# UW-RoboSoccer/tsid_control

Measured on AMD Instinct MI355X. Metric: env-steps/sec (whole node), higher is better.
Workload: dtype f64

## Files before the change

### tsid_control_amd/csrc/tsidb_common.hpp

```cpp
#pragma once
#include <hip/hip_runtime.h>
#include <stdint.h>

#ifdef TSIDB_STAMPS
constexpr int NSTAMP = 48;
__device__ unsigned long long g_stamp[8192][NSTAMP];
#define TSIDB_STAMP(k) do { if (threadIdx.x == 0 && blockIdx.x < 8192) g_stamp[blockIdx.x][k] = __builtin_amdgcn_s_memtime(); } while (0)
#define TSIDB_LAP_INIT() unsigned long long lap_t_ = __builtin_amdgcn_s_memtime()
#define TSIDB_LAP(k) do { unsigned long long n_ = __builtin_amdgcn_s_memtime(); if (threadIdx.x == 0 && blockIdx.x < 8192) g_stamp[blockIdx.x][k] += n_ - lap_t_; lap_t_ = n_; } while (0)
#define TSIDB_LAP_ZERO(k) do { if (threadIdx.x == 0 && blockIdx.x < 8192) g_stamp[blockIdx.x][k] = 0; } while (0)
#else
#define TSIDB_STAMP(k) do { } while (0)
#define TSIDB_LAP_INIT() do { } while (0)
#define TSIDB_LAP(k) do { } while (0)
#define TSIDB_LAP_ZERO(k) do { } while (0)
#endif

#ifndef TSIDB_TOPOLOGY_HEADER
#define TSIDB_TOPOLOGY_HEADER "tsidb_topology.hpp"
#endif
#include TSIDB_TOPOLOGY_HEADER

namespace tsidb {

// ... 159 lines not shown
  s = (q & 2) ? -s0 : s0;
  c = ((q + 1) & 2) ? -c0 : c0;
}

__device__ __forceinline__ int env_of_block(int b, int n) {
  constexpr int NXCD = 8;
  const int x = b % NXCD, i = b / NXCD, q = n / NXCD, r = n % NXCD;
  return x * q + (x < r ? x : r) + i;
}

constexpr double SIM_STATE_BOUND = 1e6;
template <typename T> struct Eps;
template <> struct Eps<double> { static constexpr double v = 2.220446049250313e-16; static constexpr double inf = 1e300; };
template <> struct Eps<float> { static constexpr float v = 1.1920929e-07f; static constexpr float inf = 1e30f; };

template <int CTRL, int ROW_MASK> __device__ __forceinline__ float dpp_mov(float v) {
  return __builtin_bit_cast(float, __builtin_amdgcn_update_dpp(0, __builtin_bit_cast(int, v), CTRL, ROW_MASK, 0xf, true));
}
template <int CTRL, int ROW_MASK> __device__ __forceinline__ double dpp_mov(double v) {
  const long long b = __builtin_bit_cast(long long, v);
  const int lo = __builtin_amdgcn_update_dpp(0, (int)(b & 0xffffffffLL), CTRL, ROW_MASK, 0xf, true);
  const int hi = __builtin_amdgcn_update_dpp(0, (int)(b >> 32), CTRL, ROW_MASK, 0xf, true);
  return __builtin_bit_cast(double, ((long long)hi << 32) | (unsigned int)lo);
}
__device__ __forceinline__ float lane63(float v) {
  return __builtin_bit_cast(float, __builtin_amdgcn_readlane(__builtin_bit_cast(int, v), 63));
}
__device__ __forceinline__ int lane63(int v) { return __builtin_amdgcn_readlane(v, 63); }
__device__ __forceinline__ double lane63(double v) {
  const long long b = __builtin_bit_cast(long long, v);
  const int lo = __builtin_amdgcn_readlane((int)(b & 0xffffffffLL), 63), hi = __builtin_amdgcn_readlane((int)(b >> 32), 63);
  return __builtin_bit_cast(double, ((long long)hi << 32) | (unsigned int)lo);
}
template <typename T> __device__ __forceinline__ T wave_sum(T v) {
  v += dpp_mov<0xB1, 0xf>(v);
  v += dpp_mov<0x4E, 0xf>(v);
  v += dpp_mov<0x141, 0xf>(v);
  v += dpp_mov<0x140, 0xf>(v);
  v += dpp_mov<0x142, 0xa>(v);
  v += dpp_mov<0x143, 0xc>(v);
  return lane63(v);
}
template <typename T> __device__ __forceinline__ void wave_sum3(T &a, T &b, T &c) {
#define TSIDB_SUM3_STEP(CTRL, MASK)                                                                  \
  {                                                                                                  \
    const T ta = dpp_mov<CTRL, MASK>(a), tb = dpp_mov<CTRL, MASK>(b), tc = dpp_mov<CTRL, MASK>(c);   \
    a += ta; b += tb; c += tc;                                                                       \
  }
  TSIDB_SUM3_STEP(0xB1, 0xf) TSIDB_SUM3_STEP(0x4E, 0xf) TSIDB_SUM3_STEP(0x141, 0xf) TSIDB_SUM3_STEP(0x140, 0xf)
  TSIDB_SUM3_STEP(0x142, 0xa) TSIDB_SUM3_STEP(0x143, 0xc)
#undef TSIDB_SUM3_STEP
  a = lane63(a); b = lane63(b); c = lane63(c);
}
template <typename T> __device__ __forceinline__ T bperm(T v, int src_lane) {
  if constexpr (sizeof(T) == 4) {
    return __builtin_bit_cast(T, __builtin_amdgcn_ds_bpermute(src_lane << 2, __builtin_bit_cast(int, v)));
  } else {
    const long long b = __builtin_bit_cast(long long, v);
    const int lo = __builtin_amdgcn_ds_bpermute(src_lane << 2, (int)(b & 0xffffffffLL));
    const int hi = __builtin_amdgcn_ds_bpermute(src_lane << 2, (int)(b >> 32));
    return __builtin_bit_cast(T, ((long long)hi << 32) | (unsigned int)lo);
  }
}
template <typename T> __device__ __forceinline__ T subtree_sum32(T v, int last) {
  T p = v;
  p += dpp_mov<0x111, 0xf>(p);
  p += dpp_mov<0x112, 0xf>(p);
  p += dpp_mov<0x114, 0xf>(p);
  p += dpp_mov<0x118, 0xf>(p);
  p += dpp_mov<0x142, 0xa>(p);
  return (bperm(p, last) - p) + v;
}

__device__ __forceinline__ int wave_sum_int(int v) {
  v += __builtin_amdgcn_update_dpp(0, v, 0xB1, 0xf, 0xf, true);
  v += __builtin_amdgcn_update_dpp(0, v, 0x4E, 0xf, 0xf, true);
  v += __builtin_amdgcn_update_dpp(0, v, 0x141, 0xf, 0xf, true);
  v += __builtin_amdgcn_update_dpp(0, v, 0x140, 0xf, 0xf, true);
  v += __builtin_amdgcn_update_dpp(0, v, 0x142, 0xa, 0xf, true);
  v += __builtin_amdgcn_update_dpp(0, v, 0x143, 0xc, 0xf, true);
  return __builtin_amdgcn_readlane(v, 63);
}

template <int CTRL, int ROW_MASK, typename T> __device__ __forceinline__ T dpp_min_step(T v) {
  T w;
  if constexpr (sizeof(T) == 4) {
    w = __builtin_bit_cast(T, __builtin_amdgcn_update_dpp(__builtin_bit_cast(int, v), __builtin_bit_cast(int, v), CTRL, ROW_MASK, 0xf, false));
  } else {
    const long long b = __builtin_bit_cast(long long, v);
    const int lo = __builtin_amdgcn_update_dpp((int)(b & 0xffffffffLL), (int)(b & 0xffffffffLL), CTRL, ROW_MASK, 0xf, false);
    const int hi = __builtin_amdgcn_update_dpp((int)(b >> 32), (int)(b >> 32), CTRL, ROW_MASK, 0xf, false);
    w = __builtin_bit_cast(T, ((long long)hi << 32) | (unsigned int)lo);
  }
  return w < v ? w : v;
}
template <typename T> __device__ __forceinline__ T wave_min(T v) {
  v = dpp_min_step<0xB1, 0xf>(v);
  v = dpp_min_step<0x4E, 0xf>(v);
  v = dpp_min_step<0x141, 0xf>(v);
  v = dpp_min_step<0x140, 0xf>(v);
  v = dpp_min_step<0x142, 0xa>(v);
  v = dpp_min_step<0x143, 0xc>(v);
  return lane63(v);
}
template <typename T> __device__ __forceinline__ void wave_argmin(T &v, int &i) {
  const T vmin = wave_min(v);
  i = wave_min<int>(v == vmin ? i : 0x7fffffff);
  v = vmin;
}
__device__ __forceinline__ int wave_min_int(int v) { return wave_min<int>(v); }

template <typename T> __device__ __forceinline__ void quat_to_R(T x, T y, T z, T w, T *R) {
  T n = T(1) / sqrt(x * x + y * y + z * z + w * w);
  x *= n; y *= n; z *= n; w *= n;
  R[0] = 1 - 2 * (y * y + z * z); R[1] = 2 * (x * y - w * z); R[2] = 2 * (x * z + w * y);
  R[3] = 2 * (x * y + w * z); R[4] = 1 - 2 * (x * x + z * z); R[5] = 2 * (y * z - w * x);
  R[6] = 2 * (x * z - w * y); R[7] = 2 * (y * z + w * x); R[8] = 1 - 2 * (x * x + y * y);
}

template <typename T> __device__ __forceinline__ void yo_mul(const T *Y, const T *X, T *f) {
  T wxh[3], hxl[3];
  cross3(X + 3, Y + 1, wxh);
  cross3(Y + 1, X, hxl);
  f[0] = Y[0] * X[0] + wxh[0];
  f[1] = Y[0] * X[1] + wxh[1];
  f[2] = Y[0] * X[2] + wxh[2];
  f[3] = Y[4] * X[3] + Y[5] * X[4] + Y[6] * X[5] + hxl[0];
  f[4] = Y[5] * X[3] + Y[7] * X[4] + Y[8] * X[5] + hxl[1];
  f[5] = Y[6] * X[3] + Y[8] * X[4] + Y[9] * X[5] + hxl[2];
}
template <typename T> __device__ __forceinline__ void cross_mm(const T *a, const T *b, T *o) {
  T t1[3], t2[3], t3[3];
  cross3(a + 3, b, t1); cross3(a, b + 3, t2); cross3(a + 3, b + 3, t3);
#pragma unroll
  for (int i = 0; i < 3; i++) { o[i] = t1[i] + t2[i]; o[3 + i] = t3[i]; }
}
template <typename T> __device__ __forceinline__ void cross_mf(const T *v, const T *f, T *o) {
  T t1[3], t2[3], t3[3];
  cross3(v + 3, f, t1); cross3(v + 3, f + 3, t2); cross3(v, f, t3);
#pragma unroll
  for (int i = 0; i < 3; i++) { o[i] = t1[i]; o[3 + i] = t2[i] + t3[i]; }
}

__device__ __forceinline__ void wave_sync() {
  __builtin_amdgcn_fence(__ATOMIC_RELEASE, "wavefront");
  __builtin_amdgcn_wave_barrier();
  __builtin_amdgcn_fence(__ATOMIC_ACQUIRE, "wavefront");
}

template <typename T>
__device__ __forceinline__ void tree_forward(int lane, int n, int up0, int up1, int up2, const int (&chn)[7], T *bufA, T *bufB,
                                             T *sq, int sq_stride, T *cb, int cb_stride, T (&R)[9], T (&p)[3], T qd,
                                             T (&S)[6], T (&V)[6], T (&A)[6]) {
  const bool on = lane < n;
  if (on) {
#pragma unroll
    for (int i = 0; i < 9; i++) bufA[lane * 12 + i] = R[i];
#pragma unroll
    for (int i = 0; i < 3; i++) bufA[lane * 12 + 9 + i] = p[i];
  }
  __syncthreads();
#pragma unroll
  for (int r = 0; r < 3; r++) {
    const int u = r == 0 ? up0 : (r == 1 ? up1 : up2);
    const T *src = (r & 1) ? bufB : bufA;
    T *dst = (r & 1) ? bufA : bufB;
// ... 112 lines not shown
```

### tsid_control_amd/csrc/tsidb_sim.hpp

```cpp
#pragma once
#include "tsidb_common.hpp"
#include "tsidb_tick.hpp"

namespace tsidb {

constexpr int LDM = 27;
constexpr int NEWTON_INCR_MAX = 8;

template <typename T>
struct Floor {
  T n[3], t1[3], t2[3], d;
};

template <typename T>
struct SimLds {
  Floor<T> fl;
  T S[NV][6];
  union {
    struct { T V[NB][6], A[NB][6], f[NB][6], Yc[NB][10]; };
    struct {
      T K[NB][21];
      T hn[MAXHH][3];
      int hb1[MAXHH];
    };
  };
  T M[NV * LDM];
  union {
    struct {
      T R[NB][9], p[NB][3];
      int fcand[64];
      int pcand[128];
      T terr[20];
      T scen[NG][4];
      T hn_s[MAXHH][3];
      int hb1_s[MAXHH];
    };
    T H[NV * LDM];
    T Wc[MAXCON][21];
  };
  T qpos[NQ], qvel[NV];
  T xv[NV];
  int cbody[MAXCON], cvert[MAXCON], cgeom[MAXCON];
  T ctq[CONDIM > 3 ? MAXCON : 1][3];
  unsigned anc[NB];
  T cr[MAXCON][3], cdist[MAXCON], cfv[MAXCON][3];
  int xch[4];
  unsigned char cchain[MAXCON][8];
};
static_assert(sizeof(SimLds<double>) <= 20480, "k_sim must fit 8 workgroups per CU");

template <int NW> __device__ __forceinline__ void wsync() {
  if constexpr (NW == 1) __syncthreads();
  else wave_sync();
}

__device__ __forceinline__ int sym_idx(int i, int j) {
  const int a = i < j ? i : j, b = i < j ? j : i;
  return a * 6 - a * (a - 1) / 2 + (b - a);
}

template <typename T, bool DENSE>
__device__ __forceinline__ T chol26_solve(T (&a)[NV], T rhs, int lane, bool &spd) {
  int ln = lane;
  asm volatile("" : "+v"(ln));
  int notspd = 0;
  T rd[NV];
#pragma unroll
  for (int t = 0; t < NV; t++) {
    const int k = NV - 1 - t;
    const T akk = rdlane(a[k], k);
    notspd = akk > 0 ? notspd : 1;
    asm volatile("" : "+v"(notspd));
    const T rk = rsqrt_t(akk > 0 ? akk : T(1));
    rd[k] = rk;
    T uik = ln < k ? a[k] * rk : (ln == k ? akk * rk : T(0));
    a[k] = uik;
    int jl = -1;
#pragma unroll
    for (int j0 = 0; j0 < k; j0 += 4) {
      const bool p0 = DENSE || ((MJ_DOFANC[k] >> j0) & 1u), p1 = j0 + 1 < k && (DENSE || ((MJ_DOFANC[k] >> (j0 + 1)) & 1u)),
                 p2 = j0 + 2 < k && (DENSE || ((MJ_DOFANC[k] >> (j0 + 2)) & 1u)), p3 = j0 + 3 < k && (DENSE || ((MJ_DOFANC[k] >> (j0 + 3)) & 1u));
      if (!(p0 || p1 || p2 || p3)) continue;
      const T u0 = p0 ? rdlane(uik, j0) : T(0), u1 = p1 ? rdlane(uik, j0 + 1) : T(0), u2 = p2 ? rdlane(uik, j0 + 2) : T(0),
              u3 = p3 ? rdlane(uik, j0 + 3) : T(0);
      if (jl >= 0) asm volatile("" : "+v"(uik), "+v"(a[jl]) : "s"(u0), "s"(u1), "s"(u2), "s"(u3));
      else asm volatile("" : "+v"(uik) : "s"(u0), "s"(u1), "s"(u2), "s"(u3));
      if (p0) { a[j0] -= uik * u0; jl = j0; }
      if (p1) { a[j0 + 1] -= uik * u1; jl = j0 + 1; }
      if (p2) { a[j0 + 2] -= uik * u2; jl = j0 + 2; }
      if (p3) { a[j0 + 3] -= uik * u3; jl = j0 + 3; }
    }
  }
  spd = notspd == 0;
#pragma unroll
  for (int k = 0; k < NV; k++) asm volatile("" : "+v"(a[k]));
  T acc = rhs, y[NV];
#pragma unroll
  for (int t = 0; t < NV; t++) {
    const int k = NV - 1 - t;
    y[k] = rdlane(acc, k) * rd[k];
    acc -= a[k] * y[k];
  }
  T xs[NV], x = 0;
#pragma unroll
  for (int t = NV - 1; t >= 0; t--) {
    const int k = NV - 1 - t;
    T s0 = y[k], s1 = 0, ak = a[k];
#pragma unroll
    for (int i0 = 0; i0 < k; i0 += 4) {
      const bool p0 = DENSE || ((MJ_DOFANC[k] >> i0) & 1u), p1 = i0 + 1 < k && (DENSE || ((MJ_DOFANC[k] >> (i0 + 1)) & 1u)),
                 p2 = i0 + 2 < k && (DENSE || ((MJ_DOFANC[k] >> (i0 + 2)) & 1u)), p3 = i0 + 3 < k && (DENSE || ((MJ_DOFANC[k] >> (i0 + 3)) & 1u));
      if (!(p0 || p1 || p2 || p3)) continue;
      const T u0 = p0 ? rdlane(ak, i0) : T(0), u1 = p1 ? rdlane(ak, i0 + 1) : T(0), u2 = p2 ? rdlane(ak, i0 + 2) : T(0),
              u3 = p3 ? rdlane(ak, i0 + 3) : T(0);
      asm volatile("" : "+v"(ak), "+v"(s0), "+v"(s1) : "s"(u0), "s"(u1), "s"(u2), "s"(u3));
      if (p0) s0 -= u0 * xs[i0];
      if (p1) s1 -= u1 * xs[i0 + 1];
      if (p2) s0 -= u2 * xs[i0 + 2];
      if (p3) s1 -= u3 * xs[i0 + 3];
    }
    xs[k] = (s0 + s1) * rd[k];
    if (ln == k) x = xs[k];
  }
  return x;
}

template <typename T>
__device__ __noinline__ T chol26_dense(T (&a)[NV], T rhs, int lane, bool &spd) { return chol26_solve<T, true>(a, rhs, lane, spd); }

template <typename T>
__device__ __forceinline__ void chol26_factor(T (&a)[NV], T &rdv, int lane, bool &spd) {
  int ln = lane;
  asm volatile("" : "+v"(ln));
  int notspd = 0;
  rdv = 0;
#pragma unroll
  for (int t = 0; t < NV; t++) {
    const int k = NV - 1 - t;
    const T akk = rdlane(a[k], k);
    notspd = akk > 0 ? notspd : 1;
    asm volatile("" : "+v"(notspd));
    const T rk = rsqrt_t(akk > 0 ? akk : T(1));
    rdv = ln == k ? rk : rdv;
    T uik = ln < k ? a[k] * rk : (ln == k ? akk * rk : T(0));
    a[k] = uik;
    int jl = -1;
#pragma unroll
    for (int j0 = 0; j0 < k; j0 += 4) {
      const bool p0 = (MJ_DOFANC[k] >> j0) & 1u, p1 = j0 + 1 < k && ((MJ_DOFANC[k] >> (j0 + 1)) & 1u),
                 p2 = j0 + 2 < k && ((MJ_DOFANC[k] >> (j0 + 2)) & 1u), p3 = j0 + 3 < k && ((MJ_DOFANC[k] >> (j0 + 3)) & 1u);
      if (!(p0 || p1 || p2 || p3)) continue;
      const T u0 = p0 ? rdlane(uik, j0) : T(0), u1 = p1 ? rdlane(uik, j0 + 1) : T(0), u2 = p2 ? rdlane(uik, j0 + 2) : T(0),
              u3 = p3 ? rdlane(uik, j0 + 3) : T(0);
      if (jl >= 0) asm volatile("" : "+v"(uik), "+v"(a[jl]) : "s"(u0), "s"(u1), "s"(u2), "s"(u3));
      else asm volatile("" : "+v"(uik) : "s"(u0), "s"(u1), "s"(u2), "s"(u3));
      if (p0) { a[j0] -= uik * u0; jl = j0; }
      if (p1) { a[j0 + 1] -= uik * u1; jl = j0 + 1; }
      if (p2) { a[j0 + 2] -= uik * u2; jl = j0 + 2; }
      if (p3) { a[j0 + 3] -= uik * u3; jl = j0 + 3; }
    }
  }
  spd = notspd == 0;
#pragma unroll
  for (int k = 0; k < NV; k++) asm volatile("" : "+v"(a[k]));
}

template <typename T>
__device__ __forceinline__ T chol26_subst(const T (&a)[NV], const T *Up, T rdv, T rhs, int lane) {
  int ln = lane;
  asm volatile("" : "+v"(ln));
  T b[NV];
#pragma unroll
  for (int i = 0; i < NV; i++) b[i] = lane < NV ? Up[i * LDM + lane] : T(0);
  T acc = rhs, yv = 0;
#pragma unroll
  for (int t = 0; t < NV; t++) {
    const int k = NV - 1 - t;
    const T yl = acc * rdv;
    const T yk = rdlane(yl, k);
    yv = ln == k ? yl : yv;
    acc -= a[k] * yk;
  }
  acc = yv;
  T x = 0;
#pragma unroll
  for (int i = 0; i < NV; i++) {
    const T xl = acc * rdv;
    const T xi = rdlane(xl, i);
    x = ln == i ? xl : x;
    acc -= b[i] * xi;
  }
  return x;
}

template <typename T>
__device__ __forceinline__ bool chol26_rank1(T (&a)[NV], T &rdv, T xv, T sigma, unsigned long long chain, int lane) {
  bool ok = true;
#pragma unroll
  for (int t = 0; t < NV; t++) {
    const int k = NV - 1 - t;
    if (ok && ((chain >> k) & 1ull)) {
      const T s = rdlane(xv * rdv, k);
      const T q = T(1) + sigma * s * s;
      if (!(q > (sizeof(T) == 8 ? T(1e-10) : T(1e-5)))) ok = false;
      else {
        const T ic = rsqrt_t(q), c = q * ic;
        const T un = (a[k] + sigma * s * xv) * ic;
        xv = lane == k ? T(0) : c * xv - s * un;
        a[k] = un;
        rdv = lane == k ? rdv * ic : rdv;
      }
    }
  }
  return ok;
}

template <typename T> __device__ __forceinline__ T mulM(const SimLds<T> &L, const T *x, int lane) {
  T s = 0, s1 = 0, s2 = 0, s3 = 0;
  if (lane < NV) {
    const T *Mr = &L.M[lane * LDM];
#pragma unroll
    for (int j = 0; j < NV; j += 4) {
      s += Mr[j] * x[j];
      if (j + 1 < NV) s1 += Mr[j + 1] * x[j + 1];
      if (j + 2 < NV) s2 += Mr[j + 2] * x[j + 2];
      if (j + 3 < NV) s3 += Mr[j + 3] * x[j + 3];
    }
  }
  return (s + s1) + (s2 + s3);
}

template <typename T> __device__ __forceinline__ void make_frame(const T *n, T *t1, T *t2) {
  T t[3] = {0, 0, 0};
  if (fabs(n[1]) < T(0.5)) t[1] = 1; else t[2] = 1;
  const T dn = dot3(n, t);
  T nn = 0;
#pragma unroll
  for (int i = 0; i < 3; i++) { t1[i] = t[i] - dn * n[i]; nn += t1[i] * t1[i]; }
  nn = T(1) / sqrt(nn);
#pragma unroll
  for (int i = 0; i < 3; i++) t1[i] *= nn;
  cross3(n, t1, t2);
// ... 1676 lines not shown
```

### tsid_control_amd/csrc/tsidb_tick.hpp

```cpp
#pragma once
#include "tsidb_common.hpp"

namespace tsidb {

constexpr int NAS = 34;

template <typename T>
struct KinScratch {
  T S[NV][6], fR[2][9], fp[2][3];
  union {
    T f[NJ][6];
    struct { T arhs[4][6], acomr[3], apost[NA], aamr[3]; };
  };
  T Yc[NJ][10];
  union {
    struct { T R[NJ][9], p[NJ][3], V[NJ][6], A[NJ][6]; };
    struct { T Jf[12 * LDF], Jcom[3 * LDF], Jam[3 * LDF]; };
  };
};

template <typename T>
struct ActiveSetLds {
  T Ra[NAS * (NAS + 1) / 2 + 2];
  T Rinv[NAS + 2];
  T s[160];
  T actp[3][NA];
  int slot[NAS + 2], A[NAS + 2], Aold[NAS + 2];
  unsigned char cstate[160];
};

template <typename T>
struct TickLds {
  union {
    KinScratch<T> k;
    ActiveSetLds<T> as;
  };
  T Dyn[NV * LDD];
  T h[NV];
  T x[NVAR];
  T oMf[2][12];
  T vf[2][6], af[2][6];
  T com[3], vcom[3], acomd[3];
  T Lam[3], dLam[3];
  T qs[NQ], vs[NV];
  int act[2];
};
static_assert(sizeof(ActiveSetLds<double>) <= sizeof(KinScratch<double>), "active-set state must fit the scratch region");
static_assert(sizeof(TickLds<double>) <= 20480, "k_tick must fit 8 workgroups per CU");

template <typename T> __device__ __forceinline__ T bcast(T v, int src) { return __shfl(v, src, WAVE); }

__device__ __forceinline__ float rdlane(float v, int src) {
  return __builtin_bit_cast(float, __builtin_amdgcn_readlane(__builtin_bit_cast(int, v), src));
}
__device__ __forceinline__ double rdlane(double v, int src) {
  long long b = __builtin_bit_cast(long long, v);
  int lo = __builtin_amdgcn_readlane((int)(b & 0xffffffffLL), src);
  int hi = __builtin_amdgcn_readlane((int)(b >> 32), src);
  return __builtin_bit_cast(double, ((long long)hi << 32) | (unsigned int)lo);
}


template <typename T>
__device__ __forceinline__ void rbd_terms(const DevModel<T> &m, TickLds<T> &L, int lane) {
  KinScratch<T> &K = L.k;
  const T GZ = T(9.81);
  TSIDB_LAP_ZERO(15); TSIDB_LAP_ZERO(23); TSIDB_LAP_ZERO(29); TSIDB_LAP_ZERO(30); TSIDB_LAP_ZERO(31);
  TSIDB_LAP_INIT();
  for (int i = lane; i < NV * LDD; i += WAVE) L.Dyn[i] = 0;
  T Rj[9], pj[3], Vj[6], Aj[6], Sj[6], qd = 0;
  const int up0 = lane < NJ ? m.pin_up[0][lane] : -1, up1 = lane < NJ ? m.pin_up[1][lane] : -1,
            up2 = lane < NJ ? m.pin_up[2][lane] : -1;
  int jchn[7];
#pragma unroll
  for (int d = 0; d < 7; d++) jchn[d] = lane < NJ ? m.pin_chain[lane][d] : -1;
  const int fpar0 = m.frame_parent[0], fpar1 = m.frame_parent[1];
  const unsigned fanc0 = m.pin_anc[fpar0], fanc1 = m.pin_anc[fpar1];
#pragma unroll
  for (int i = 0; i < 6; i++) { Vj[i] = 0; Aj[i] = 0; Sj[i] = 0; }
#pragma unroll
  for (int i = 0; i < 3; i++) pj[i] = 0;
#pragma unroll
  for (int i = 0; i < 9; i++) Rj[i] = 0;
  if (lane == 0) {
    quat_to_R(L.qs[3], L.qs[4], L.qs[5], L.qs[6], Rj);
    mat3vec(Rj, &L.vs[0], Vj);
    mat3vec(Rj, &L.vs[3], Vj + 3);
#pragma unroll
    for (int k = 0; k < 3; k++) {
#pragma unroll
      for (int i = 0; i < 3; i++) {
        K.S[k][i] = Rj[3 * i + k]; K.S[k][3 + i] = 0;
        K.S[3 + k][i] = 0; K.S[3 + k][3 + i] = Rj[3 * i + k];
      }
    }
  } else if (lane < NJ) {
    const T *PR = m.pin_place[lane];
    const T th = L.qs[6 + lane];
    T c, s;
    sincos_t(th, s, c);
    qd = L.vs[5 + lane];
#pragma unroll
    for (int i = 0; i < 3; i++) {
      Rj[3 * i + 0] = c * PR[3 * i] + s * PR[3 * i + 1];
      Rj[3 * i + 1] = -s * PR[3 * i] + c * PR[3 * i + 1];
      Rj[3 * i + 2] = PR[3 * i + 2];
      pj[i] = PR[9 + i];
    }
  }
  TSIDB_LAP(15);
  tree_forward<T>(lane, NJ, up0, up1, up2, jchn, &K.R[0][0], &K.V[0][0], &K.f[0][0], 6, &K.Yc[0][0], 10, Rj, pj, qd, Sj,
                  Vj, Aj);
  if (lane < NJ) {
    const int j = lane;
    if (j > 0) {
#pragma unroll
      for (int i = 0; i < 6; i++) K.S[5 + j][i] = Sj[i];
    }
#pragma unroll
    for (int i = 0; i < 9; i++) K.R[j][i] = Rj[i];
#pragma unroll
    for (int i = 0; i < 3; i++) K.p[j][i] = pj[i];
#pragma unroll
    for (int i = 0; i < 6; i++) { K.V[j][i] = Vj[i]; K.A[j][i] = Aj[i]; }
  }
  TSIDB_LAP(23);
  {
    T fb[6] = {0, 0, 0, 0, 0, 0}, Y[10] = {0, 0, 0, 0, 0, 0, 0, 0, 0, 0};
    if (lane < NJ) {
      const int j = lane;
      const T *Yb = m.pin_inertia[j];
      T cw[3], I[9] = {Yb[4], Yb[5], Yb[6], Yb[5], Yb[7], Yb[8], Yb[6], Yb[8], Yb[9]}, Tm[9], RT[9];
      mat3vec(Rj, Yb + 1, cw);
#pragma unroll
      for (int i = 0; i < 3; i++) cw[i] += pj[i];
      mat3mul(Rj, I, Tm);
#pragma unroll
      for (int i = 0; i < 3; i++)
#pragma unroll
        for (int k = 0; k < 3; k++) RT[3 * i + k] = Rj[3 * k + i];
      mat3mul(Tm, RT, I);
      T mass = Yb[0], c2 = dot3(cw, cw);
      Y[0] = mass; Y[1] = mass * cw[0]; Y[2] = mass * cw[1]; Y[3] = mass * cw[2];
      Y[4] = I[0] + mass * (c2 - cw[0] * cw[0]); Y[5] = I[1] - mass * cw[0] * cw[1]; Y[6] = I[2] - mass * cw[0] * cw[2];
// ... 1032 lines not shown
                 com_ref[6 + i] - L.acomd[i];
  } else if (lane < 10) {
    const int i = lane - 7;
    L.k.aamr[i] = -m.params[P_KP_AM + i] * L.Lam[i] - L.dLam[i];
  } else if (lane >= 32 && lane < 32 + NA) {
    const int r = lane - 32;
    L.k.apost[r] = -m.params[P_KP_POSTURE + r] * (L.qs[7 + r] - posture_ref[r]) - m.params[P_KD_POSTURE + r] * L.vs[6 + r];
  }
  for (int idx = lane; idx < NV * 12 * c.nslot; idx += WAVE) {
    const int r = idx / (12 * c.nslot), cc = idx % (12 * c.nslot), s = cc / 12, e = cc % 12, f = slot_foot<T, NS>(L, s);
    T a = 0;
#pragma unroll
    for (int i = 0; i < 6; i++) a += m.Tgen[i][e] * L.k.Jf[(6 * f + i) * LDF + r];
    L.Dyn[r * LDD + NV + cc] = -a;
  }
  __syncthreads();
  TSIDB_STAMP(2);

  const T w_foot = m.params[P_W_FOOT], w_com = m.params[P_W_COM], w_post = m.params[P_W_POSTURE], reg = m.params[P_HESS_REG];
  T jt[15], a[NV];
  {
    const int i = lane < NV ? lane : 0;
#pragma unroll
    for (int r = 0; r < 12; r++) jt[r] = lane < NV ? L.k.Jf[r * LDF + i] : T(0);
#pragma unroll
    for (int r = 0; r < 3; r++) jt[12 + r] = lane < NV ? L.k.Jcom[r * LDF + i] : T(0);
  }
  T gi = 0;
#pragma unroll
  for (int r = 0; r < 12; r++) gi -= w_foot * jt[r] * L.k.arhs[2 + r / 6][r % 6];
#pragma unroll
  for (int r = 0; r < 3; r++) gi -= w_com * jt[12 + r] * L.k.acomr[r];
  if (lane >= 6 && lane < NV) gi -= w_post * L.k.apost[lane - 6];
  {
    T wjt[15];
#pragma unroll
    for (int r = 0; r < 12; r++) wjt[r] = w_foot * jt[r];
#pragma unroll
    for (int r = 0; r < 3; r++) wjt[12 + r] = w_com * jt[12 + r];
#pragma unroll
    for (int j = 0; j < NV; j++) {
      T acc = 0, acc1 = 0;
#pragma unroll
      for (int r = 0; r < 12; r++) {
        if (r & 1) acc1 += wjt[r] * L.k.Jf[r * LDF + j];
        else acc += wjt[r] * L.k.Jf[r * LDF + j];
      }
#pragma unroll
      for (int r = 0; r < 3; r++) {
        if (r & 1) acc1 += wjt[12 + r] * L.k.Jcom[r * LDF + j];
        else acc += wjt[12 + r] * L.k.Jcom[r * LDF + j];
      }
      a[j] = acc + acc1;
    }
  }
  const T w_am = m.params[P_W_AM];
  if (w_am != 0) {
    T ja[3];
#pragma unroll
    for (int r = 0; r < 3; r++) ja[r] = lane < NV ? L.k.Jam[r * LDF + (lane < NV ? lane : 0)] : T(0);
#pragma unroll
    for (int r = 0; r < 3; r++) gi -= w_am * ja[r] * L.k.aamr[r];
#pragma unroll
    for (int j = 0; j < NV; j++) {
      T acc = 0;
#pragma unroll
      for (int r = 0; r < 3; r++) acc += w_am * ja[r] * rdlane(ja[r], j);
      a[j] += acc;
    }
  }
  if (lane >= NV) gi = 0;
  int ln = lane;
  asm volatile("" : "+v"(ln));
  T dg = 0;
#pragma unroll
  for (int j = 0; j < NV; j++)
    if (ln == j) { a[j] += reg + (j >= 6 ? w_post : T(0)); dg = a[j]; }
  T c1 = wave_sum(dg) + T(c.nslot) * m.Hf_trace;

  int qp_status = -1, qp_iters = 0;
  TSIDB_STAMP(3);
  T rdv = 0;
  int notspd = 0;
  asm volatile("" : "+v"(ln));
#pragma unroll
  for (int k = 0; k < NV; k++) {
    const T akk = rdlane(a[k], k);
    notspd = akk > 0 ? notspd : 1;
    asm volatile("" : "+v"(notspd));
    const T rk = rsqrt_t(akk > 0 ? akk : T(1));
    if (ln == k) rdv = rk;
    const T lik = ln == k ? akk * rk : a[k] * rk;
    a[k] = lik;
    T lk = lik;
#pragma unroll
    for (int j0 = k + 1; j0 < NV; j0 += 4) {
      const bool p1 = j0 + 1 < NV, p2 = j0 + 2 < NV, p3 = j0 + 3 < NV;
      const T u0 = rdlane(lk, j0), u1 = p1 ? rdlane(lk, p1 ? j0 + 1 : 0) : T(0), u2 = p2 ? rdlane(lk, p2 ? j0 + 2 : 0) : T(0),
              u3 = p3 ? rdlane(lk, p3 ? j0 + 3 : 0) : T(0);
      if (j0 > k + 1) asm volatile("" : "+v"(lk), "+v"(a[j0 - 1]) : "s"(u0), "s"(u1), "s"(u2), "s"(u3));
      else asm volatile("" : "+v"(lk) : "s"(u0), "s"(u1), "s"(u2), "s"(u3));
      a[j0] -= lk * u0;
      if (p1) a[j0 + 1] -= lk * u1;
      if (p2) a[j0 + 2] -= lk * u2;
      if (p3) a[j0 + 3] -= lk * u3;
    }
  }
  TSIDB_STAMP(4);
#pragma unroll
  for (int k = 0; k < NV; k++) asm volatile("" : "+v"(a[k]));
  const bool spd = notspd == 0;
  tick_qp<T, NS, COP>(m, L, c, lane, a, rdv, gi, c1, spd, cop_ref, qp_status, qp_iters, fast_eq);
  int status = qp_status, iters = qp_iters;

  TSIDB_STAMP(8);
  const bool solved = status == 0;
  if (lane < NV) dv[lane] = solved ? L.x[lane] : T(0);
  if (lane < 24) {
    const int fo = lane / 12, e = lane % 12;
    T val = 0;
    for (int s = 0; s < c.nslot; s++)
      if (solved && slot_foot<T, NS>(L, s) == fo) val = L.x[NV + 12 * s + e];
    fout[lane] = val;
    L.as.s[lane] = val;
  }
  T tau2 = 0;
  if (lane < NA) {
    constexpr int NNc = NV + 12 * NS;
    const T *Dr = &L.Dyn[(6 + lane) * LDD];
    T t = L.h[6 + lane], t1 = 0, t2 = 0, t3 = 0;
#pragma unroll
    for (int e = 0; e < NNc; e += 4) {
      t += Dr[e] * L.x[e];
      if (e + 1 < NNc) t1 += Dr[e + 1] * L.x[e + 1];
      if (e + 2 < NNc) t2 += Dr[e + 2] * L.x[e + 2];
      if (e + 3 < NNc) t3 += Dr[e + 3] * L.x[e + 3];
    }
    t = (t + t1) + (t2 + t3);
    if (m.params[P_FRICTION_COMP] != 0) {
      const T vn = L.vs[6 + lane] + m.params[P_DT] * L.x[6 + lane], sat = vn * T(20);
      t += m.params[P_FRICTION_COMP] * (sat > 1 ? T(1) : (sat < -1 ? T(-1) : sat));
    }
    t = solved ? t : T(0);
    tau[lane] = t;
    tau2 = t * t;
  }
  if (rowx) tau2 = wave_sum(tau2);
  if (lane == 0) {
    status_out[0] = status;
    if (info) { info[0] = iters; info[1] = c.iq; }
  }
  __syncthreads();
  if (obs) {
    T wl = 0;
    if (lane < 12) {
      const int fo = lane / 6, i = lane % 6;
#pragma unroll
      for (int e = 0; e < 12; e++) wl += m.Tgen[i][e] * L.as.s[12 * fo + e];
    }
    T fz[2], copw[2][3];
#pragma unroll
    for (int fo = 0; fo < 2; fo++) {
      const T w2 = rdlane(wl, 6 * fo + 2), w3 = rdlane(wl, 6 * fo + 3), w4 = rdlane(wl, 6 * fo + 4);
      T cl[3] = {0, 0, 0};
      const bool on = L.act[fo] != 0;
      if (on && w2 > T(1e-3)) { cl[0] = w4 / w2; cl[1] = w3 / w2; }
      const T *F = (m.params[P_QUIRKS] != 0 && cop_frames) ? cop_frames + 12 * fo : L.oMf[fo];
#pragma unroll
      for (int i = 0; i < 3; i++) copw[fo][i] = F[3 * i] * cl[0] + F[3 * i + 1] * cl[1] + F[3 * i + 2] * cl[2] + F[9 + i];
      fz[fo] = w2;
    }
    T cop[3] = {0, 0, 0};
    if (NS == 2 && fz[0] + fz[1] != 0) {
      cop[0] = (copw[0][0] * fz[0] + copw[1][0] * fz[1]) / (fz[0] + fz[1]);
      cop[1] = (copw[0][1] * fz[0] + copw[1][1] * fz[1]) / (fz[0] + fz[1]);
    }
    if (lane < 3) obs[NQ + NV + 3 + lane] = lane == 0 ? cop[0] : (lane == 1 ? cop[1] : cop[2]);
    if (lane >= 8 && lane < 11) obs[NQ + NV + lane - 8] = L.com[lane - 8];
    if (lane >= 16 && lane < 19) obs[NQ + NV + 6 + lane - 16] = L.oMf[0][9 + lane - 16];
    if (lane >= 24 && lane < 27) obs[NQ + NV + 9 + lane - 24] = L.oMf[1][9 + lane - 24];
  }
  if (status == 0) {
    const T dt = m.params[P_DT];
    T vm = 0;
    if (lane < NV) {
      const T vv = L.vs[lane], dd = L.x[lane];
      vm = dt * (vv + T(0.5) * dt * dd);
      L.vs[lane] = vv + dt * dd;
      L.as.Ra[lane] = vm;
    }
// ... 59 lines not shown
```

Before: 18.74 million.

## Use DPP row_newbcast FMAs for f64 Cholesky rank-1 updates instead of readlane

```diff
diff --git a/tsid_control_amd/csrc/tsidb_common.hpp b/tsid_control_amd/csrc/tsidb_common.hpp
--- a/tsid_control_amd/csrc/tsidb_common.hpp
+++ b/tsid_control_amd/csrc/tsidb_common.hpp
@@ -265,6 +265,88 @@
   return __builtin_amdgcn_readlane(v, 63);
 }
 
+template <int K> struct IntC { static constexpr int value = K; };
+template <int K0, int K1, typename F> __device__ __forceinline__ void unroll_for(F &&f) {
+  if constexpr (K0 < K1) { f(IntC<K0>{}); unroll_for<K0 + 1, K1>(f); }
+}
+struct RowDup { double lo, hi; };
+typedef unsigned tsidb_v2u_t __attribute__((ext_vector_type(2)));
+__device__ __forceinline__ RowDup row_dup(double x) {
+  const unsigned long long v = __builtin_bit_cast(unsigned long long, x);
+  const tsidb_v2u_t l = __builtin_amdgcn_permlane16_swap((unsigned)v, (unsigned)v, false, false);
+  const tsidb_v2u_t h = __builtin_amdgcn_permlane16_swap((unsigned)(v >> 32), (unsigned)(v >> 32), false, false);
+  RowDup d;
+  d.lo = __builtin_bit_cast(double, ((unsigned long long)h[0] << 32) | l[0]);
+  d.hi = __builtin_bit_cast(double, ((unsigned long long)h[1] << 32) | l[1]);
+  return d;
+}
+constexpr int mask_bit_at(unsigned mask, int n) {
+  int r = -1;
+  for (int b = 0; b < 32; b++)
+    if ((mask >> b) & 1u) { if (n == 0 && r < 0) r = b; n--; }
+  return r;
+}
+constexpr int mask_count(unsigned mask) { int c = 0; for (; mask; mask &= mask - 1) c++; return c; }
+constexpr unsigned mask_drop_low(unsigned mask, int n) { for (; n > 0 && mask; n--) mask &= mask - 1; return mask; }
+#define TSIDB_BF(i) "v_fmac_f64_dpp %[a" #i "], -%[x" #i "], %[m] row_newbcast:%[j" #i "] row_mask:0xf bank_mask:0xf\n"
+#define TSIDB_BO(i) [a##i] "+v"(a[mask_bit_at(MASK, i)])
+#define TSIDB_BI(i) [x##i] "v"(mask_bit_at(MASK, i) < 16 ? d.lo : d.hi), [j##i] "n"(mask_bit_at(MASK, i) & 15)
+template <unsigned MASK, int N> __device__ __forceinline__ void bcast_fnma(double (&a)[N], const RowDup &d, double m) {
+  constexpr int C = mask_count(MASK);
+  static_assert(N >= 32 || (MASK >> (N & 31)) == 0u, "lanes of the accumulator array");
+  if constexpr (C == 1) asm volatile("s_nop 1\n" TSIDB_BF(0) : TSIDB_BO(0) : [m] "v"(m), TSIDB_BI(0));
+  else if constexpr (C == 2) asm volatile("s_nop 1\n" TSIDB_BF(0) TSIDB_BF(1) : TSIDB_BO(0), TSIDB_BO(1) : [m] "v"(m), TSIDB_BI(0), TSIDB_BI(1));
+  else if constexpr (C == 3)
+    asm volatile("s_nop 1\n" TSIDB_BF(0) TSIDB_BF(1) TSIDB_BF(2) : TSIDB_BO(0), TSIDB_BO(1), TSIDB_BO(2) : [m] "v"(m), TSIDB_BI(0), TSIDB_BI(1), TSIDB_BI(2));
+  else if constexpr (C == 4)
+    asm volatile("s_nop 1\n" TSIDB_BF(0) TSIDB_BF(1) TSIDB_BF(2) TSIDB_BF(3)
+                 : TSIDB_BO(0), TSIDB_BO(1), TSIDB_BO(2), TSIDB_BO(3)
+                 : [m] "v"(m), TSIDB_BI(0), TSIDB_BI(1), TSIDB_BI(2), TSIDB_BI(3));
+  else if constexpr (C == 5)
+    asm volatile("s_nop 1\n" TSIDB_BF(0) TSIDB_BF(1) TSIDB_BF(2) TSIDB_BF(3) TSIDB_BF(4)
+                 : TSIDB_BO(0), TSIDB_BO(1), TSIDB_BO(2), TSIDB_BO(3), TSIDB_BO(4)
+                 : [m] "v"(m), TSIDB_BI(0), TSIDB_BI(1), TSIDB_BI(2), TSIDB_BI(3), TSIDB_BI(4));
+  else if constexpr (C == 6)
+    asm volatile("s_nop 1\n" TSIDB_BF(0) TSIDB_BF(1) TSIDB_BF(2) TSIDB_BF(3) TSIDB_BF(4) TSIDB_BF(5)
+                 : TSIDB_BO(0), TSIDB_BO(1), TSIDB_BO(2), TSIDB_BO(3), TSIDB_BO(4), TSIDB_BO(5)
+                 : [m] "v"(m), TSIDB_BI(0), TSIDB_BI(1), TSIDB_BI(2), TSIDB_BI(3), TSIDB_BI(4), TSIDB_BI(5));
+  else if constexpr (C == 7)
+    asm volatile("s_nop 1\n" TSIDB_BF(0) TSIDB_BF(1) TSIDB_BF(2) TSIDB_BF(3) TSIDB_BF(4) TSIDB_BF(5) TSIDB_BF(6)
+                 : TSIDB_BO(0), TSIDB_BO(1), TSIDB_BO(2), TSIDB_BO(3), TSIDB_BO(4), TSIDB_BO(5), TSIDB_BO(6)
+                 : [m] "v"(m), TSIDB_BI(0), TSIDB_BI(1), TSIDB_BI(2), TSIDB_BI(3), TSIDB_BI(4), TSIDB_BI(5), TSIDB_BI(6));
+  else if constexpr (C >= 8) {
+    asm volatile("s_nop 1\n" TSIDB_BF(0) TSIDB_BF(1) TSIDB_BF(2) TSIDB_BF(3) TSIDB_BF(4) TSIDB_BF(5) TSIDB_BF(6) TSIDB_BF(7)
+                 : TSIDB_BO(0), TSIDB_BO(1), TSIDB_BO(2), TSIDB_BO(3), TSIDB_BO(4), TSIDB_BO(5), TSIDB_BO(6), TSIDB_BO(7)
+                 : [m] "v"(m), TSIDB_BI(0), TSIDB_BI(1), TSIDB_BI(2), TSIDB_BI(3), TSIDB_BI(4), TSIDB_BI(5), TSIDB_BI(6), TSIDB_BI(7));
+    bcast_fnma<mask_drop_low(MASK, 8)>(a, d, m);
+  }
+}
+#undef TSIDB_BF
+#undef TSIDB_BO
+#undef TSIDB_BI
+#define TSIDB_BF(c, i, sg) ".if %[n" c "] > " #i "\nv_fmac_f64_dpp %[" c "], " sg "%[x" c #i "], %[m" c #i "] row_newbcast:%[j" c #i "] row_mask:0xf bank_mask:0xf\n.endif\n"
+#define TSIDB_BI(c, M, i) [x##c##i] "v"(mask_bit_at(M, i) >= 16 ? d.hi : d.lo), [m##c##i] "v"(m[mask_bit_at(M, i) < 0 ? 0 : mask_bit_at(M, i)]), \
+                          [j##c##i] "n"(mask_bit_at(M, i) < 0 ? 0 : (mask_bit_at(M, i) & 15))
+#define TSIDB_BG(sg)                                                                                                              \
+  asm volatile("s_nop 1\n" TSIDB_BF("e", 0, sg) TSIDB_BF("o", 0, sg) TSIDB_BF("e", 1, sg) TSIDB_BF("o", 1, sg)                    \
+               TSIDB_BF("e", 2, sg) TSIDB_BF("o", 2, sg) TSIDB_BF("e", 3, sg) TSIDB_BF("o", 3, sg)                                \
+               : [e] "+v"(s0), [o] "+v"(s1)                                                                                       \
+               : [ne] "n"(CE), [no] "n"(CO), TSIDB_BI(e, E, 0), TSIDB_BI(o, O, 0), TSIDB_BI(e, E, 1), TSIDB_BI(o, O, 1),          \
+                 TSIDB_BI(e, E, 2), TSIDB_BI(o, O, 2), TSIDB_BI(e, E, 3), TSIDB_BI(o, O, 3))
+template <unsigned MASK, int N>
+__device__ __forceinline__ void bcast_fnma2(double &s0, double &s1, const RowDup &d, const double (&m)[N]) {
+  static_assert(N >= 32 || (MASK >> (N & 31)) == 0u, "lanes of the multiplier array");
+  constexpr unsigned E = MASK & 0x55555555u, O = MASK & 0xaaaaaaaau;
+  constexpr int CE = mask_count(E) < 4 ? mask_count(E) : 4, CO = mask_count(O) < 4 ? mask_count(O) : 4;
+  if constexpr (MASK != 0u) {
+    TSIDB_BG("-");
+    bcast_fnma2<mask_drop_low(E, 4) | mask_drop_low(O, 4)>(s0, s1, d, m);
+  }
+}
+#undef TSIDB_BF
+#undef TSIDB_BI
+#undef TSIDB_BG
+
 template <int CTRL, int ROW_MASK, typename T> __device__ __forceinline__ T dpp_min_step(T v) {
   T w;
   if constexpr (sizeof(T) == 4) {
diff --git a/tsid_control_amd/csrc/tsidb_sim.hpp b/tsid_control_amd/csrc/tsidb_sim.hpp
--- a/tsid_control_amd/csrc/tsidb_sim.hpp
+++ b/tsid_control_amd/csrc/tsidb_sim.hpp
@@ -65,30 +65,43 @@
   asm volatile("" : "+v"(ln));
   int notspd = 0;
   T rd[NV];
-#pragma unroll
-  for (int t = 0; t < NV; t++) {
-    const int k = NV - 1 - t;
+  auto pivot = [&](int k) __attribute__((always_inline)) -> T {
     const T akk = rdlane(a[k], k);
     notspd = akk > 0 ? notspd : 1;
     asm volatile("" : "+v"(notspd));
     const T rk = rsqrt_t(akk > 0 ? akk : T(1));
     rd[k] = rk;
-    T uik = ln < k ? a[k] * rk : (ln == k ? akk * rk : T(0));
+    const T uik = ln < k ? a[k] * rk : (ln == k ? akk * rk : T(0));
     a[k] = uik;
-    int jl = -1;
-#pragma unroll
-    for (int j0 = 0; j0 < k; j0 += 4) {
-      const bool p0 = DENSE || ((MJ_DOFANC[k] >> j0) & 1u), p1 = j0 + 1 < k && (DENSE || ((MJ_DOFANC[k] >> (j0 + 1)) & 1u)),
-                 p2 = j0 + 2 < k && (DENSE || ((MJ_DOFANC[k] >> (j0 + 2)) & 1u)), p3 = j0 + 3 < k && (DENSE || ((MJ_DOFANC[k] >> (j0 + 3)) & 1u));
-      if (!(p0 || p1 || p2 || p3)) continue;
-      const T u0 = p0 ? rdlane(uik, j0) : T(0), u1 = p1 ? rdlane(uik, j0 + 1) : T(0), u2 = p2 ? rdlane(uik, j0 + 2) : T(0),
-              u3 = p3 ? rdlane(uik, j0 + 3) : T(0);
-      if (jl >= 0) asm volatile("" : "+v"(uik), "+v"(a[jl]) : "s"(u0), "s"(u1), "s"(u2), "s"(u3));
-      else asm volatile("" : "+v"(uik) : "s"(u0), "s"(u1), "s"(u2), "s"(u3));
-      if (p0) { a[j0] -= uik * u0; jl = j0; }
-      if (p1) { a[j0 + 1] -= uik * u1; jl = j0 + 1; }
-      if (p2) { a[j0 + 2] -= uik * u2; jl = j0 + 2; }
-      if (p3) { a[j0 + 3] -= uik * u3; jl = j0 + 3; }
+    return uik;
+  };
+  if constexpr (!DENSE && sizeof(T) == 8) {
+    unroll_for<0, NV>([&](auto tt) {
+      constexpr int k = NV - 1 - decltype(tt)::value;
+      const T uik = pivot(k);
+      constexpr unsigned ANC = MJ_DOFANC[k] & ((1u << k) - 1u);
+      if constexpr (ANC != 0u) bcast_fnma<ANC>(a, row_dup(uik), uik);
+    });
+  } else {
+#pragma unroll
+    for (int t = 0; t < NV; t++) {
+      const int k = NV - 1 - t;
+      T uik = pivot(k);
+      int jl = -1;
+#pragma unroll
+      for (int j0 = 0; j0 < k; j0 += 4) {
+        const bool p0 = DENSE || ((MJ_DOFANC[k] >> j0) & 1u), p1 = j0 + 1 < k && (DENSE || ((MJ_DOFANC[k] >> (j0 + 1)) & 1u)),
+                   p2 = j0 + 2 < k && (DENSE || ((MJ_DOFANC[k] >> (j0 + 2)) & 1u)), p3 = j0 + 3 < k && (DENSE || ((MJ_DOFANC[k] >> (j0 + 3)) & 1u));
+        if (!(p0 || p1 || p2 || p3)) continue;
+        const T u0 = p0 ? rdlane(uik, j0) : T(0), u1 = p1 ? rdlane(uik, j0 + 1) : T(0), u2 = p2 ? rdlane(uik, j0 + 2) : T(0),
+                u3 = p3 ? rdlane(uik, j0 + 3) : T(0);
+        if (jl >= 0) asm volatile("" : "+v"(uik), "+v"(a[jl]) : "s"(u0), "s"(u1), "s"(u2), "s"(u3));
+        else asm volatile("" : "+v"(uik) : "s"(u0), "s"(u1), "s"(u2), "s"(u3));
+        if (p0) { a[j0] -= uik * u0; jl = j0; }
+        if (p1) { a[j0 + 1] -= uik * u1; jl = j0 + 1; }
+        if (p2) { a[j0 + 2] -= uik * u2; jl = j0 + 2; }
+        if (p3) { a[j0 + 3] -= uik * u3; jl = j0 + 3; }
+      }
     }
   }
   spd = notspd == 0;
@@ -102,25 +115,36 @@
     acc -= a[k] * y[k];
   }
   T xs[NV], x = 0;
-#pragma unroll
-  for (int t = NV - 1; t >= 0; t--) {
-    const int k = NV - 1 - t;
-    T s0 = y[k], s1 = 0, ak = a[k];
-#pragma unroll
-    for (int i0 = 0; i0 < k; i0 += 4) {
-      const bool p0 = DENSE || ((MJ_DOFANC[k] >> i0) & 1u), p1 = i0 + 1 < k && (DENSE || ((MJ_DOFANC[k] >> (i0 + 1)) & 1u)),
-                 p2 = i0 + 2 < k && (DENSE || ((MJ_DOFANC[k] >> (i0 + 2)) & 1u)), p3 = i0 + 3 < k && (DENSE || ((MJ_DOFANC[k] >> (i0 + 3)) & 1u));
-      if (!(p0 || p1 || p2 || p3)) continue;
-      const T u0 = p0 ? rdlane(ak, i0) : T(0), u1 = p1 ? rdlane(ak, i0 + 1) : T(0), u2 = p2 ? rdlane(ak, i0 + 2) : T(0),
-              u3 = p3 ? rdlane(ak, i0 + 3) : T(0);
-      asm volatile("" : "+v"(ak), "+v"(s0), "+v"(s1) : "s"(u0), "s"(u1), "s"(u2), "s"(u3));
-      if (p0) s0 -= u0 * xs[i0];
-      if (p1) s1 -= u1 * xs[i0 + 1];
-      if (p2) s0 -= u2 * xs[i0 + 2];
-      if (p3) s1 -= u3 * xs[i0 + 3];
-    }
-    xs[k] = (s0 + s1) * rd[k];
-    if (ln == k) x = xs[k];
+  if constexpr (!DENSE && sizeof(T) == 8) {
+    unroll_for<0, NV>([&](auto kk) {
+      constexpr int k = decltype(kk)::value;
+      T s0 = y[k], s1 = 0;
+      constexpr unsigned ANC = MJ_DOFANC[k] & ((1u << k) - 1u);
+      if constexpr (ANC != 0u) bcast_fnma2<ANC>(s0, s1, row_dup(a[k]), xs);
+      xs[k] = (s0 + s1) * rd[k];
+      if (ln == k) x = xs[k];
+    });
+  } else {
+#pragma unroll
+    for (int t = NV - 1; t >= 0; t--) {
+      const int k = NV - 1 - t;
+      T s0 = y[k], s1 = 0, ak = a[k];
+#pragma unroll
+      for (int i0 = 0; i0 < k; i0 += 4) {
+        const bool p0 = DENSE || ((MJ_DOFANC[k] >> i0) & 1u), p1 = i0 + 1 < k && (DENSE || ((MJ_DOFANC[k] >> (i0 + 1)) & 1u)),
+                   p2 = i0 + 2 < k && (DENSE || ((MJ_DOFANC[k] >> (i0 + 2)) & 1u)), p3 = i0 + 3 < k && (DENSE || ((MJ_DOFANC[k] >> (i0 + 3)) & 1u));
+        if (!(p0 || p1 || p2 || p3)) continue;
+        const T u0 = p0 ? rdlane(ak, i0) : T(0), u1 = p1 ? rdlane(ak, i0 + 1) : T(0), u2 = p2 ? rdlane(ak, i0 + 2) : T(0),
+                u3 = p3 ? rdlane(ak, i0 + 3) : T(0);
+        asm volatile("" : "+v"(ak), "+v"(s0), "+v"(s1) : "s"(u0), "s"(u1), "s"(u2), "s"(u3));
+        if (p0) s0 -= u0 * xs[i0];
+        if (p1) s1 -= u1 * xs[i0 + 1];
+        if (p2) s0 -= u2 * xs[i0 + 2];
+        if (p3) s1 -= u3 * xs[i0 + 3];
+      }
+      xs[k] = (s0 + s1) * rd[k];
+      if (ln == k) x = xs[k];
+    }
   }
   return x;
 }
@@ -134,30 +158,43 @@
   asm volatile("" : "+v"(ln));
   int notspd = 0;
   rdv = 0;
-#pragma unroll
-  for (int t = 0; t < NV; t++) {
-    const int k = NV - 1 - t;
+  auto pivot = [&](int k) __attribute__((always_inline)) -> T {
     const T akk = rdlane(a[k], k);
     notspd = akk > 0 ? notspd : 1;
     asm volatile("" : "+v"(notspd));
     const T rk = rsqrt_t(akk > 0 ? akk : T(1));
     rdv = ln == k ? rk : rdv;
-    T uik = ln < k ? a[k] * rk : (ln == k ? akk * rk : T(0));
+    const T uik = ln < k ? a[k] * rk : (ln == k ? akk * rk : T(0));
     a[k] = uik;
-    int jl = -1;
-#pragma unroll
-    for (int j0 = 0; j0 < k; j0 += 4) {
-      const bool p0 = (MJ_DOFANC[k] >> j0) & 1u, p1 = j0 + 1 < k && ((MJ_DOFANC[k] >> (j0 + 1)) & 1u),
-                 p2 = j0 + 2 < k && ((MJ_DOFANC[k] >> (j0 + 2)) & 1u), p3 = j0 + 3 < k && ((MJ_DOFANC[k] >> (j0 + 3)) & 1u);
-      if (!(p0 || p1 || p2 || p3)) continue;
-      const T u0 = p0 ? rdlane(uik, j0) : T(0), u1 = p1 ? rdlane(uik, j0 + 1) : T(0), u2 = p2 ? rdlane(uik, j0 + 2) : T(0),
-              u3 = p3 ? rdlane(uik, j0 + 3) : T(0);
-      if (jl >= 0) asm volatile("" : "+v"(uik), "+v"(a[jl]) : "s"(u0), "s"(u1), "s"(u2), "s"(u3));
-      else asm volatile("" : "+v"(uik) : "s"(u0), "s"(u1), "s"(u2), "s"(u3));
-      if (p0) { a[j0] -= uik * u0; jl = j0; }
-      if (p1) { a[j0 + 1] -= uik * u1; jl = j0 + 1; }
-      if (p2) { a[j0 + 2] -= uik * u2; jl = j0 + 2; }
-      if (p3) { a[j0 + 3] -= uik * u3; jl = j0 + 3; }
+    return uik;
+  };
+  if constexpr (sizeof(T) == 8) {
+    unroll_for<0, NV>([&](auto tt) {
+      constexpr int k = NV - 1 - decltype(tt)::value;
+      const T uik = pivot(k);
+      constexpr unsigned ANC = MJ_DOFANC[k] & ((1u << k) - 1u);
+      if constexpr (ANC != 0u) bcast_fnma<ANC>(a, row_dup(uik), uik);
+    });
+  } else {
+#pragma unroll
+    for (int t = 0; t < NV; t++) {
+      const int k = NV - 1 - t;
+      T uik = pivot(k);
+      int jl = -1;
+#pragma unroll
+      for (int j0 = 0; j0 < k; j0 += 4) {
+        const bool p0 = (MJ_DOFANC[k] >> j0) & 1u, p1 = j0 + 1 < k && ((MJ_DOFANC[k] >> (j0 + 1)) & 1u),
+                   p2 = j0 + 2 < k && ((MJ_DOFANC[k] >> (j0 + 2)) & 1u), p3 = j0 + 3 < k && ((MJ_DOFANC[k] >> (j0 + 3)) & 1u);
+        if (!(p0 || p1 || p2 || p3)) continue;
+        const T u0 = p0 ? rdlane(uik, j0) : T(0), u1 = p1 ? rdlane(uik, j0 + 1) : T(0), u2 = p2 ? rdlane(uik, j0 + 2) : T(0),
+                u3 = p3 ? rdlane(uik, j0 + 3) : T(0);
+        if (jl >= 0) asm volatile("" : "+v"(uik), "+v"(a[jl]) : "s"(u0), "s"(u1), "s"(u2), "s"(u3));
+        else asm volatile("" : "+v"(uik) : "s"(u0), "s"(u1), "s"(u2), "s"(u3));
+        if (p0) { a[j0] -= uik * u0; jl = j0; }
+        if (p1) { a[j0 + 1] -= uik * u1; jl = j0 + 1; }
+        if (p2) { a[j0 + 2] -= uik * u2; jl = j0 + 2; }
+        if (p3) { a[j0 + 3] -= uik * u3; jl = j0 + 3; }
+      }
     }
   }
   spd = notspd == 0;
diff --git a/tsid_control_amd/csrc/tsidb_tick.hpp b/tsid_control_amd/csrc/tsidb_tick.hpp
--- a/tsid_control_amd/csrc/tsidb_tick.hpp
+++ b/tsid_control_amd/csrc/tsidb_tick.hpp
@@ -60,6 +60,44 @@
   return __builtin_bit_cast(double, ((long long)hi << 32) | (unsigned int)lo);
 }
 
+template <typename T, bool DPPB> __device__ __forceinline__ void tick_chol(T (&a)[NV], T &rdv, int &notspd, int &ln) {
+  static_assert(!DPPB || sizeof(T) == 8, "the DPP form is float64 only");
+  asm volatile("" : "+v"(ln));
+  auto pivot = [&](int k) __attribute__((always_inline)) -> T {
+    const T akk = rdlane(a[k], k);
+    notspd = akk > 0 ? notspd : 1;
+    asm volatile("" : "+v"(notspd));
+    const T rk = rsqrt_t(akk > 0 ? akk : T(1));
+    if (ln == k) rdv = rk;
+    const T lik = ln == k ? akk * rk : a[k] * rk;
+    a[k] = lik;
+    return lik;
+  };
+  if constexpr (DPPB) {
+    unroll_for<0, NV>([&](auto kk) {
+      constexpr int k = decltype(kk)::value;
+      const T lik = pivot(k);
+      if constexpr (k + 1 < NV) bcast_fnma<((1u << NV) - 1u) & ~((2u << k) - 1u)>(a, row_dup(lik), lik);
+    });
+  } else {
+#pragma unroll
+    for (int k = 0; k < NV; k++) {
+      T lk = pivot(k);
+#pragma unroll
+      for (int j0 = k + 1; j0 < NV; j0 += 4) {
+        const bool p1 = j0 + 1 < NV, p2 = j0 + 2 < NV, p3 = j0 + 3 < NV;
+        const T u0 = rdlane(lk, j0), u1 = p1 ? rdlane(lk, p1 ? j0 + 1 : 0) : T(0), u2 = p2 ? rdlane(lk, p2 ? j0 + 2 : 0) : T(0),
+                u3 = p3 ? rdlane(lk, p3 ? j0 + 3 : 0) : T(0);
+        if (j0 > k + 1) asm volatile("" : "+v"(lk), "+v"(a[j0 - 1]) : "s"(u0), "s"(u1), "s"(u2), "s"(u3));
+        else asm volatile("" : "+v"(lk) : "s"(u0), "s"(u1), "s"(u2), "s"(u3));
+        a[j0] -= lk * u0;
+        if (p1) a[j0 + 1] -= lk * u1;
+        if (p2) a[j0 + 2] -= lk * u2;
+        if (p3) a[j0 + 3] -= lk * u3;
+      }
+    }
+  }
+}
 
 template <typename T>
 __device__ __forceinline__ void rbd_terms(const DevModel<T> &m, TickLds<T> &L, int lane) {
@@ -1258,30 +1296,7 @@
   TSIDB_STAMP(3);
   T rdv = 0;
   int notspd = 0;
-  asm volatile("" : "+v"(ln));
-#pragma unroll
-  for (int k = 0; k < NV; k++) {
-    const T akk = rdlane(a[k], k);
-    notspd = akk > 0 ? notspd : 1;
-    asm volatile("" : "+v"(notspd));
-    const T rk = rsqrt_t(akk > 0 ? akk : T(1));
-    if (ln == k) rdv = rk;
-    const T lik = ln == k ? akk * rk : a[k] * rk;
-    a[k] = lik;
-    T lk = lik;
-#pragma unroll
-    for (int j0 = k + 1; j0 < NV; j0 += 4) {
-      const bool p1 = j0 + 1 < NV, p2 = j0 + 2 < NV, p3 = j0 + 3 < NV;
-      const T u0 = rdlane(lk, j0), u1 = p1 ? rdlane(lk, p1 ? j0 + 1 : 0) : T(0), u2 = p2 ? rdlane(lk, p2 ? j0 + 2 : 0) : T(0),
-              u3 = p3 ? rdlane(lk, p3 ? j0 + 3 : 0) : T(0);
-      if (j0 > k + 1) asm volatile("" : "+v"(lk), "+v"(a[j0 - 1]) : "s"(u0), "s"(u1), "s"(u2), "s"(u3));
-      else asm volatile("" : "+v"(lk) : "s"(u0), "s"(u1), "s"(u2), "s"(u3));
-      a[j0] -= lk * u0;
-      if (p1) a[j0 + 1] -= lk * u1;
-      if (p2) a[j0 + 2] -= lk * u2;
-      if (p3) a[j0 + 3] -= lk * u3;
-    }
-  }
+  tick_chol<T, sizeof(T) == 8>(a, rdv, notspd, ln);
   TSIDB_STAMP(4);
 #pragma unroll
   for (int k = 0; k < NV; k++) asm volatile("" : "+v"(a[k]));
```

Result: faster. 19.34 million, median of 6 (+3.2%).
